# Bojian-Wei/Non-IID-Distributed-Learning-with-Optimal-Mixture-Weights

Hardware: AMD Instinct MI355X
Metric: client-rounds/sec (whole node) (higher is better)
Workload: dtype f32; 1 GPU; config 2: fedavg, 100 clients x 512 rows, RFF D=2048, C=10, E=2, B=32, 10000 test rows, round=1880, parallel clients; algo=fedavg, clients_total=100, clients_per_gpu=100, rows_per_client=512, D=2048, C=10, epochs=2, batch=32, test_rows=10000, parallelism=clients1

## Files before the change

### non-iid-distributed-learning-with-optimal-mixture-weights_amd/_lib.py

```python
import ctypes as C
import os

import torch

from . import LIB_PATH

_c_f32p = C.POINTER(C.c_float)
_SIGS = {
    'fs_abi_version': (C.c_int, []),
    'fs_last_error': (C.c_char_p, []),
    'fs_tuning_size': (C.c_int64, []),
    'fs_set_tuning': (C.c_int, [C.c_void_p]),
    'fs_set_thread_tuning': (C.c_int, [C.c_void_p]),
    'fs_get_tuning': (C.c_int, [C.c_void_p]),
    'fs_get_process_tuning': (C.c_int, [C.c_void_p]),
    'fs_get_thread_tuning': (C.c_int, [C.c_void_p]),
    'fs_randperm_batch': (C.c_int, [C.c_void_p, C.c_void_p, C.c_void_p, C.c_int64, C.c_void_p, C.c_int]),
    'fs_libsvm_scan': (C.c_int, [C.c_char_p, C.c_void_p, C.c_void_p, C.c_void_p]),
    'fs_libsvm_read': (C.c_int, [C.c_char_p, C.c_int64, C.c_int64, C.c_int, C.c_void_p, C.c_void_p, C.c_int]),
    'fs_randperm_device': (C.c_int, [C.c_void_p, C.c_void_p, C.c_void_p, C.c_int64, C.c_int64, C.c_void_p,
                                     C.c_void_p, C.c_void_p]),
    'fs_local_train_plan': (C.c_int, [C.c_int, C.c_int, C.c_int, C.c_int, C.c_int64, C.c_int64, C.c_int,
                                      C.c_int, C.c_void_p, C.c_void_p]),
    'fs_local_train': (C.c_int, [C.c_void_p, C.c_int64, C.c_void_p, C.c_void_p, C.c_void_p, C.c_void_p,
                                 C.c_int, C.c_int, C.c_int, C.c_int, C.c_float, C.c_float, C.c_int,
                                 C.c_float, C.c_int, C.c_int, C.c_void_p, C.c_void_p, C.c_void_p,
                                 C.c_int, C.c_void_p, C.c_int64, C.c_void_p]),
    'fs_local_train_mse': (C.c_int, [C.c_void_p, C.c_int64, C.c_void_p, C.c_void_p, C.c_void_p, C.c_void_p,
                                     C.c_int, C.c_int, C.c_int, C.c_float, C.c_float, C.c_int, C.c_float, C.c_int,
                                     C.c_int, C.c_void_p, C.c_void_p, C.c_void_p, C.c_void_p]),
    'fs_aggregate': (C.c_int, [C.c_void_p, C.c_int64, C.c_void_p, C.c_int, C.c_int64, C.c_void_p,
                               C.c_void_p, C.c_int64, C.c_int, C.c_void_p]),
    'fs_aggregate_sel': (C.c_int, [C.c_void_p, C.c_int64, C.c_void_p, C.c_void_p, C.c_int, C.c_int64, C.c_void_p,
                                   C.c_void_p, C.c_int64, C.c_int, C.c_void_p]),
    'fs_aggregate_nova': (C.c_int, [C.c_void_p, C.c_int64, C.c_void_p, C.c_void_p, C.c_void_p, C.c_float, C.c_float,
                                    C.c_int, C.c_void_p, C.c_int, C.c_int64, C.c_void_p, C.c_void_p, C.c_int64,
                                    C.c_int, C.c_void_p]),
    'fs_local_train_scaffold': (C.c_int, [C.c_void_p, C.c_int64, C.c_void_p, C.c_void_p, C.c_void_p, C.c_void_p,
                                          C.c_int, C.c_int, C.c_int, C.c_int, C.c_float, C.c_float, C.c_int,
                                          C.c_void_p, C.c_void_p, C.c_void_p, C.c_void_p, C.c_void_p, C.c_void_p]),
    'fs_aggregate_scaffold': (C.c_int, [C.c_void_p, C.c_int64, C.c_void_p, C.c_void_p, C.c_void_p, C.c_float, C.c_int,
                                        C.c_int64, C.c_void_p, C.c_void_p, C.c_void_p, C.c_int64, C.c_int, C.c_void_p]),
    'fs_plan_set_scaffold': (C.c_int, [C.c_void_p, C.c_int, C.c_void_p, C.c_void_p, C.c_void_p, C.c_float]),
    'fs_aggregate_opt': (C.c_int, [C.c_void_p, C.c_int64, C.c_void_p, C.c_void_p, C.c_int, C.c_float, C.c_float,
                                   C.c_float, C.c_float, C.c_float, C.c_float, C.c_int, C.c_int64, C.c_void_p,
                                   C.c_void_p, C.c_void_p, C.c_void_p, C.c_int64, C.c_int, C.c_void_p]),
    'fs_plan_set_server_opt': (C.c_int, [C.c_void_p, C.c_int, C.c_void_p, C.c_void_p, C.c_float, C.c_float, C.c_float,
                                         C.c_float, C.c_float, C.c_float]),
    'fs_eval_ws_doubles': (C.c_int64, [C.c_int]),
    'fs_eval': (C.c_int, [C.c_void_p, C.c_int64, C.c_void_p, C.c_int, C.c_void_p, C.c_int, C.c_void_p,
                          C.c_void_p, C.c_void_p]),
    'fs_eval_mse': (C.c_int, [C.c_void_p, C.c_int64, C.c_void_p, C.c_int, C.c_void_p, C.c_void_p, C.c_void_p,
                              C.c_void_p]),
    'fs_z_eval_block_rows': (C.c_int, []),
    'fs_z_eval_ws_doubles': (C.c_int64, [C.c_int, C.c_int]),
    'fs_z_eval_add': (C.c_int, [C.c_void_p, C.c_void_p, C.c_int, C.c_int, C.c_int, C.c_int, C.c_int, C.c_void_p,
                                C.c_int64, C.c_void_p]),
    'fs_z_eval_add_mse': (C.c_int, [C.c_void_p, C.c_void_p, C.c_int, C.c_int, C.c_int, C.c_int, C.c_void_p,
                                    C.c_int64, C.c_void_p]),
    'fs_z_eval_finish': (C.c_int, [C.c_void_p, C.c_int64, C.c_int, C.c_int, C.c_void_p, C.c_void_p]),
    'fs_eval_clients_ws_doubles': (C.c_int64, [C.c_int64, C.c_int]),
    'fs_eval_clients': (C.c_int, [C.c_void_p, C.c_int64, C.c_void_p, C.c_void_p, C.c_void_p, C.c_int, C.c_void_p,
                                  C.c_int64, C.c_int, C.c_void_p, C.c_void_p, C.c_int64, C.c_void_p]),
    'fs_eval_clients_mse': (C.c_int, [C.c_void_p, C.c_int64, C.c_void_p, C.c_void_p, C.c_void_p, C.c_int, C.c_void_p,
                                      C.c_int64, C.c_void_p, C.c_void_p, C.c_int64, C.c_void_p]),
    'fs_mix_z': (C.c_int, [C.c_void_p, C.c_void_p, C.c_int64, C.c_int, C.c_int, C.c_int, C.c_void_p,
                           C.c_void_p]),
    'fs_mix_solve_ws_bytes': (C.c_int64, [C.c_int, C.c_int, C.c_int]),
    'fs_mix_solve': (C.c_int, [C.c_void_p, C.c_void_p, C.c_void_p, C.c_int, C.c_int, C.c_int, C.c_int,
                               C.c_int, C.c_float, C.c_float, C.c_void_p, C.c_void_p, C.c_void_p,
                               C.c_void_p, C.c_int64, C.c_void_p]),
    'fs_mix_solve_mse': (C.c_int, [C.c_void_p, C.c_void_p, C.c_void_p, C.c_int, C.c_int, C.c_int, C.c_int,
                                   C.c_float, C.c_float, C.c_void_p, C.c_void_p, C.c_void_p, C.c_void_p, C.c_int64,
                                   C.c_void_p]),
    'fs_mix_solve_blocked': (C.c_int, [C.c_void_p, C.c_int, C.c_void_p, C.c_void_p, C.c_int, C.c_int, C.c_int,
                                       C.c_int, C.c_int, C.c_float, C.c_float, C.c_void_p, C.c_void_p, C.c_void_p,
                                       C.c_void_p, C.c_int64, C.c_void_p]),
    'fs_mix_solve_blocked_covers': (C.c_int, [C.c_int, C.c_int, C.c_int, C.c_int, C.c_int]),
    'fs_mix_solve_last_mode': (C.c_int, []),
    'fs_mix_solve_last_layout': (C.c_int, [C.c_void_p, C.c_void_p]),
    'fs_mix_solve_plan': (C.c_int, [C.c_int, C.c_int, C.c_int, C.c_int, C.c_int, C.c_int, C.c_void_p]),
    'fs_feature_map': (C.c_int, [C.c_void_p, C.c_int64, C.c_void_p, C.c_void_p, C.c_int, C.c_int, C.c_int,
                                 C.c_float, C.c_void_p, C.c_int64, C.c_void_p]),
    'fs_gram': (C.c_int, [C.c_void_p, C.c_int64, C.c_int64, C.c_int, C.c_void_p, C.c_int64, C.c_void_p]),
    'fs_hetero': (C.c_int, [C.c_void_p, C.c_int64, C.c_void_p, C.c_int, C.c_int, C.c_void_p, C.c_int64, C.c_int64,
                            C.c_void_p, C.c_void_p]),
    'fs_plan_desc_size': (C.c_int64, []),
    'fs_plan_create': (C.c_int, [C.c_void_p, C.c_void_p]),
    'fs_plan_destroy': (C.c_int, [C.c_void_p]),
    'fs_plan_shuffle': (C.c_int, [C.c_void_p, C.c_void_p, C.c_int]),
    'fs_plan_round': (C.c_int, [C.c_void_p, C.c_int, C.c_float, C.c_int, C.c_void_p, C.c_void_p]),
    'fs_plan_eval_flush': (C.c_int, [C.c_void_p, C.c_void_p]),
    'fs_plan_shuffle_subset': (C.c_int, [C.c_void_p, C.c_void_p, C.c_void_p, C.c_int, C.c_int]),
    'fs_plan_round_subset': (C.c_int, [C.c_void_p, C.c_int, C.c_float, C.c_int, C.c_void_p, C.c_void_p, C.c_void_p,
                                       C.c_int, C.c_void_p]),
    'fs_plan_set_nova': (C.c_int, [C.c_void_p, C.c_int, C.c_void_p, C.c_float, C.c_float]),
    'fs_local_train_last_kernel': (C.c_int, []),
    'fs_plan_set_shuffle_chunk': (C.c_int, [C.c_void_p, C.c_int]),
    'fs_plan_shuffle_flush': (C.c_int, [C.c_void_p]),
    'fs_plan_eval_blocks': (C.c_int, [C.c_void_p]),
    'fs_timer_create': (C.c_int, [C.c_void_p]),
    'fs_timer_record': (C.c_int, [C.c_void_p, C.c_void_p]),
    'fs_timer_elapsed_ms': (C.c_int, [C.c_void_p, C.c_void_p, C.c_void_p]),
    'fs_timer_destroy': (C.c_int, [C.c_void_p]),
}

EXPORTS = tuple(_SIGS)
ABI_VERSION = 23

PHASE_TRAIN, PHASE_AGGREGATE, PHASE_EVAL, PHASE_EVAL_DEFER = 1, 2, 4, 8
NOVA_REFERENCE, NOVA_UPDATES = 1, 2
OPT_AVGM, OPT_ADAGRAD, OPT_ADAM, OPT_YOGI = 1, 2, 3, 4
OPT_RULES = {'avgm': OPT_AVGM, 'adagrad': OPT_ADAGRAD, 'adam': OPT_ADAM, 'yogi': OPT_YOGI}
G_PAIR = 256
G_TEAMS = 512
LT_KERNELS = {1: 'single', 2: 'split', 3: 'dbuf', 4: 'pair', 5: 'pipe', 6: 'teams', 7: 'mb',
              8: 'wide'}
G_PIPE = 1024
G_WIDE = 2048
ERR_BLOCK = 256
SOLVER_NAMES = {0: 'none', 1: 'reg', 2: 'mc', 3: 'staged', 4: 'global', 5: 'reg2', 6: 'wave', 8: 'quad', 9: 'qmc', 10: 'bin'}
SOLVERS = {v: k for k, v in SOLVER_NAMES.items() if k}


class Tuning(C.Structure):
    _fields_ = [('mix_solver', C.c_int), ('mix_prefetch', C.c_int), ('mix_prefetch_lead', C.c_int),
                ('mix_exact_softmax', C.c_int), ('no_eval_fuse', C.c_int), ('spin_limit', C.c_uint),
                ('inject_timeout', C.c_int), ('train_form', C.c_int),
                ('split_early', C.c_int), ('mix_qmc_lane_clients', C.c_int),
                ('mix_quad_loaders', C.c_int), ('split_teams', C.c_int),
                ('mix_poll_delay', C.c_int), ('split_poll_delay', C.c_int), ('split_pipe', C.c_int),
                ('split_dbuf', C.c_int),
                ('split_mb', C.c_int)]


class PlanDesc(C.Structure):
    _fields_ = [
        ('d_phi', C.c_void_p), ('ld', C.c_int64), ('d_row_off', C.c_void_p), ('d_labels', C.c_void_p),
        ('d_order', C.c_void_p), ('h_n', C.c_void_p),
        ('N', C.c_int), ('C', C.c_int), ('B', C.c_int), ('E', C.c_int), ('G', C.c_int),
        ('d_ws', C.c_void_p), ('ws_bytes', C.c_int64),
        ('chained', C.c_int), ('prox', C.c_int), ('reg', C.c_int), ('mu', C.c_float), ('lam', C.c_float),
        ('d_W_g', C.c_void_p), ('d_W_out', C.c_void_p), ('d_loss_hist', C.c_void_p),
        ('d_p', C.c_void_p), ('d_agg_ws', C.c_void_p), ('agg_ws_floats', C.c_int64), ('agg_chunks', C.c_int),
        ('d_phi_t', C.c_void_p), ('d_labels_t', C.c_void_p), ('n_t', C.c_int), ('d_eval_ws', C.c_void_p),
        ('d_eval_hist', C.c_void_p), ('shuffle_device', C.c_int), ('host_threads', C.c_int),
        ('shuffle_after_train', C.c_int),
        ('loss', C.c_int), ('d_y', C.c_void_p), ('d_y_t', C.c_void_p),
    ]

_lib = None


class FedsimError(RuntimeError):
    pass


def lib():
    global _lib
    if _lib is None:
        path = os.environ.get('FEDSIM_LIB') or LIB_PATH
        if not os.path.exists(path):
            raise FedsimError(
                'libfedsim.so not found at %s -- build it with `python -c "import __graft_entry__ as g; g.build()"` '
                'or `make -C <pkg>/csrc`; there is no CPU fallback' % path)
        h = C.CDLL(path, mode=C.RTLD_GLOBAL)
        for name, (res, args) in _SIGS.items():
            f = getattr(h, name)
            f.restype = res
            f.argtypes = args
        if h.fs_abi_version() != ABI_VERSION:
            raise FedsimError('libfedsim.so ABI %d != %d' % (h.fs_abi_version(), ABI_VERSION))
        if h.fs_tuning_size() != C.sizeof(Tuning):
            raise FedsimError('fs_tuning layout mismatch (%d != %d bytes)' % (h.fs_tuning_size(), C.sizeof(Tuning)))
        if h.fs_plan_desc_size() != C.sizeof(PlanDesc):
            raise FedsimError('fs_plan_desc layout mismatch (%d != %d bytes)' % (h.fs_plan_desc_size(),
                                                                                  C.sizeof(PlanDesc)))
        _lib = h
    return _lib


_randperm_capped = None


def randperm_device_capped():
    global _randperm_capped
    if _randperm_capped is None:
        f = getattr(lib(), '_ZN2fs15randperm_deviceEPKlS1_S1_llPiPjiPv')
        f.restype = C.c_int
        f.argtypes = [C.c_void_p, C.c_void_p, C.c_void_p, C.c_int64, C.c_int64, C.c_void_p, C.c_void_p, C.c_int,
                      C.c_void_p]
        _randperm_capped = f
    return _randperm_capped


def get_tuning():
    t = Tuning()
    check(lib().fs_get_tuning(C.byref(t)), 'fs_get_tuning')
    return {k: getattr(t, k) for k, _ in Tuning._fields_}


def last_mix_layout():
    k, nk = C.c_int(0), C.c_int(0)
    check(lib().fs_mix_solve_last_layout(C.byref(k), C.byref(nk)), 'fs_mix_solve_last_layout')
    return k.value, nk.value


class MixPlan(C.Structure):
    _fields_ = [('solver', C.c_int), ('workgroups', C.c_int), ('lane_clients', C.c_int), ('helpers', C.c_int),
                ('lead', C.c_int), ('poll_delay', C.c_int), ('ws_bytes', C.c_int64)]


def mix_plan(N, C_, n_val, epochs, Bv, blocks=1):
    out = MixPlan()
    check(lib().fs_mix_solve_plan(int(N), int(C_), int(n_val), int(epochs), int(Bv), int(blocks), C.byref(out)),
          'fs_mix_solve_plan')
    return {k: getattr(out, k) for k, _ in MixPlan._fields_}


def get_process_tuning():
    t = Tuning()
    check(lib().fs_get_process_tuning(C.byref(t)), 'fs_get_process_tuning')
    return {k: getattr(t, k) for k, _ in Tuning._fields_}


def get_thread_tuning():
    t = Tuning()
    has = lib().fs_get_thread_tuning(C.byref(t))
    if has < 0:
        check(has, 'fs_get_thread_tuning')
    return {k: getattr(t, k) for k, _ in Tuning._fields_} if has else None


def _merged(base, fields):
    cur = dict(base)
    for k, v in fields.items():
        if k not in cur:
            raise KeyError('fs_tuning has no field %r' % k)
        if k == 'mix_solver' and isinstance(v, str):
            v = 0 if v == 'auto' else SOLVERS[v]
        cur[k] = int(v)
    return cur


def set_tuning(**fields):
    prev = get_process_tuning()
    check(lib().fs_set_tuning(C.byref(Tuning(**_merged(prev, fields)))), 'fs_set_tuning')
    return prev


def set_thread_tuning(fields=None):
    if fields is None:
        check(lib().fs_set_thread_tuning(None), 'fs_set_thread_tuning')
        return
    cur = _merged({k: 0 for k, _ in Tuning._fields_}, fields)
    check(lib().fs_set_thread_tuning(C.byref(Tuning(**cur))), 'fs_set_thread_tuning')


class tuning:

    def __init__(self, **fields):
        self.fields = fields

    def __enter__(self):
        own = get_thread_tuning()
        self.thread_prev = own
        if own is not None:
            set_thread_tuning(_merged(own, self.fields))
        else:
            self.prev = set_tuning(**self.fields)
        return self

    def __exit__(self, *exc):
        if self.thread_prev is not None:
            set_thread_tuning(self.thread_prev)
        else:
            check(lib().fs_set_tuning(C.byref(Tuning(**self.prev))), 'fs_set_tuning')
        return False


def check(status, what):
    if status != 0:
        msg = lib().fs_last_error()
        raise FedsimError('%s failed (%d): %s' % (what, status, msg.decode() if msg else ''))


def ptr(t):
    return None if t is None else C.c_void_p(t.data_ptr())


def stream_ptr(stream=None):
    s = stream if stream is not None else torch.cuda.current_stream()
    return C.c_void_p(s.cuda_stream)


KERNEL_SOURCES = {
    'local_train': ('local_train.hip', 'local_train_split.hip', 'local_train_pair.hip', 'local_train_pipe.hip',
                    'local_train_dbuf.hip', 'split_common.h', 'local_train_forms.h', 'common.h',
                    'eval_rows.h', 'lanes.h'),
    'mix_solve': ('mixture.hip', 'mixture_forms.h', 'common.h', 'lanes.h'),
    'mix_z': ('mix_z.hip', 'common.h'),
    'local_train_wide': ('local_train_wide.hip', 'local_train_wide.h', 'common.h'),
    'local_train_mse': ('local_train_mse.hip', 'mse_rows.h', 'common.h'),
    'mix_solve_mse': ('mixture_mse.hip', 'mse_rows.h', 'common.h'),
    'z_eval': ('z_eval.hip', 'common.h'),
    'aggregate_nova': ('aggregate_nova.hip', 'aggregate.hip', 'aggregate_sel.h', 'finalize.h', 'common.h'),
    'local_train_scaffold': ('local_train_scaffold.hip', 'scaffold.h', 'common.h'),
    'aggregate_scaffold': ('aggregate_scaffold.hip', 'aggregate.hip', 'aggregate_sel.h', 'scaffold.h', 'finalize.h',
                           'common.h'),
    'aggregate_opt': ('aggregate_opt.hip', 'aggregate.hip', 'aggregate_sel.h', 'finalize.h', 'common.h'),
}


def source_revision(kernel=None):
    import hashlib
    import glob
    pkg = os.path.dirname(os.path.abspath(__file__))
    if kernel:
        files = sorted(os.path.join(pkg, 'csrc', f) for f in KERNEL_SOURCES[kernel])
    else:
        files = sorted(glob.glob(os.path.join(pkg, 'csrc', '*.hip')) + glob.glob(os.path.join(pkg, 'csrc', '*.h')))
    h = hashlib.sha256()
    for f in files:
        h.update(os.path.basename(f).encode())
        with open(f, 'rb') as fh:
            h.update(_code_only(fh.read().decode()).encode())
    return h.hexdigest()[:16]


_TOKENS = None


def _code_only(src):
    global _TOKENS
    import re
    if _TOKENS is None:
        _TOKENS = re.compile(r'"(?:\\.|[^"\\])*"|\'(?:\\.|[^\'\\])*\'|//[^\n]*|/\*.*?\*/|\s+|[^"\'/\s]+|/',
                             re.S)
    out = []
    for m in _TOKENS.finditer(src):
        t = m.group(0)
        if t.startswith('//') or t.startswith('/*'):
            out.append(' ')
        elif t.isspace():
            out.append(' ')
        else:
            out.append(t)
    return re.sub(r' +', ' ', ''.join(out)).strip()


class Timer:

    def __init__(self):
        self._ev = C.c_void_p()
        check(lib().fs_timer_create(C.byref(self._ev)), 'fs_timer_create')

    def record(self):
        check(lib().fs_timer_record(self._ev, stream_ptr()), 'fs_timer_record')

    def elapsed_time(self, end):
        ms = C.c_float()
        check(lib().fs_timer_elapsed_ms(self._ev, end._ev, C.byref(ms)), 'fs_timer_elapsed_ms')
        return float(ms.value)

    def __del__(self):
        if getattr(self, '_ev', None) is not None and self._ev.value and _lib is not None:
            _lib.fs_timer_destroy(self._ev)
            self._ev = None
```

### non-iid-distributed-learning-with-optimal-mixture-weights_amd/csrc/randperm.hip

```cpp
#include "common.h"
#include "randperm_geom.h"

namespace fs {

constexpr int MT_N = RP_MT_N, MT_M = 397;
constexpr int RP_THREADS = 64;

__device__ __forceinline__ uint32_t mt_mix(uint32_t a, uint32_t b, uint32_t c) {
  const uint32_t y = (a & 0x80000000u) | (b & 0x7fffffffu);
  return c ^ (y >> 1) ^ ((y & 1u) ? 0x9908b0dfu : 0u);
}

__device__ __forceinline__ uint32_t mt_temper(uint32_t y) {
  y ^= y >> 11;
  y ^= (y << 7) & 0x9d2c5680u;
  y ^= (y << 15) & 0xefc60000u;
  y ^= y >> 18;
  return y;
}

template <bool WG>
__device__ __forceinline__ void rp_sync() {
  if (WG) {
    __syncthreads();
  } else {
    asm volatile("s_waitcnt lgkmcnt(0)" ::: "memory");
    __builtin_amdgcn_wave_barrier();
    asm volatile("" ::: "memory");
  }
}

template <bool WG>
__device__ __forceinline__ void mt_twist(uint32_t* mt, int lane) {
  uint32_t v[4];
#pragma unroll
  for (int k = 0; k < 4; ++k) {
    const int i = lane + 64 * k;
    if (i < MT_N - MT_M) v[k] = mt_mix(mt[i], mt[i + 1], mt[i + MT_M]);
  }
  rp_sync<WG>();
#pragma unroll
  for (int k = 0; k < 4; ++k) {
    const int i = lane + 64 * k;
    if (i < MT_N - MT_M) mt[i] = v[k];
  }
  rp_sync<WG>();
#pragma unroll
  for (int k = 0; k < 4; ++k) {
    const int i = (MT_N - MT_M) + lane + 64 * k;
    if (i < 2 * (MT_N - MT_M)) v[k] = mt_mix(mt[i], mt[i + 1], mt[i + MT_M - MT_N]);
  }
  rp_sync<WG>();
#pragma unroll
  for (int k = 0; k < 4; ++k) {
    const int i = (MT_N - MT_M) + lane + 64 * k;
    if (i < 2 * (MT_N - MT_M)) mt[i] = v[k];
  }
  rp_sync<WG>();
#pragma unroll
  for (int k = 0; k < 3; ++k) {
    const int i = 2 * (MT_N - MT_M) + lane + 64 * k;
    if (i < MT_N - 1) v[k] = mt_mix(mt[i], mt[i + 1], mt[i + MT_M - MT_N]);
  }
  rp_sync<WG>();
#pragma unroll
  for (int k = 0; k < 3; ++k) {
    const int i = 2 * (MT_N - MT_M) + lane + 64 * k;
    if (i < MT_N - 1) mt[i] = v[k];
  }
  rp_sync<WG>();
  if (lane == 0) mt[MT_N - 1] = mt_mix(mt[MT_N - 1], mt[0], mt[MT_M - 1]);
  rp_sync<WG>();
}

__device__ __forceinline__ void rp_contract_broken(int32_t* dst, int n, int lane, int stride, uint32_t* err) {
  for (int i = lane; i < n; i += stride) dst[i] = i;
  if (err && lane == 0) __hip_atomic_store(err, 1u, __ATOMIC_RELAXED, __HIP_MEMORY_SCOPE_AGENT);
}

template <bool IN_LDS, bool WG>
__device__ __forceinline__ void rp_pass(uint32_t* mt, uint32_t* rnd, int32_t* perm_lds,
                                        const int64_t* __restrict__ seeds, const int64_t* __restrict__ ns,
                                        const int64_t* __restrict__ offs, int32_t* __restrict__ out, int64_t max_n,
                                        uint32_t* err, int64_t pass, int lane) {
  const int64_t n64 = ns[pass];
  int32_t* dst = out + offs[pass];
  if (n64 > max_n) {
    rp_contract_broken(dst, (int)n64, lane, RP_THREADS, err);
    return;
  }
  const int n = (int)n64;
  int32_t* perm = IN_LDS ? perm_lds : dst;
  for (int i = lane; i < n; i += RP_THREADS) perm[i] = i;
  if (lane == 0) {
    uint32_t x = (uint32_t)(uint64_t)seeds[pass];
    mt[0] = x;
    for (int i = 1; i < MT_N; ++i) {
      x = 1812433253u * (x ^ (x >> 30)) + (uint32_t)i;
      mt[i] = x;
    }
  }
  rp_sync<WG>();
  for (int i0 = 0; i0 < n - 1; i0 += MT_N) {
    mt_twist<WG>(mt, lane);
    for (int k = lane; k < MT_N; k += RP_THREADS) rnd[k] = mt_temper(mt[k]);
    rp_sync<WG>();
    if (lane == 0) {
      const int i1 = min(n - 1, i0 + MT_N);
      for (int i = i0; i < i1; ++i) {
        const uint32_t z = rnd[i - i0] % (uint32_t)(n - i);
        const int32_t a = perm[i];
        perm[i] = perm[i + z];
        perm[i + z] = a;
      }
    }
    rp_sync<WG>();
  }
  if (IN_LDS)
    for (int i = lane; i < n; i += RP_THREADS) dst[i] = perm[i];
}

template <bool IN_LDS>
__global__ __launch_bounds__(RP_THREADS) void randperm_kernel(const int64_t* __restrict__ seeds,
                                                             const int64_t* __restrict__ ns,
                                                             const int64_t* __restrict__ offs,
                                                             int32_t* __restrict__ out, int64_t max_n,
                                                             uint32_t* err) {
  extern __shared__ __attribute__((aligned(16))) uint32_t smem_rp[];
  uint32_t* mt = smem_rp;
  uint32_t* rnd = mt + MT_N;
  rp_pass<IN_LDS, true>(mt, rnd, reinterpret_cast<int32_t*>(rnd + MT_N), seeds, ns, offs, out, max_n, err,
                        blockIdx.x, threadIdx.x);
}

__global__ __launch_bounds__(RP_THREADS * RP_MAX_WAVES) void randperm_capped_kernel(
    const int64_t* __restrict__ seeds, const int64_t* __restrict__ ns, const int64_t* __restrict__ offs,
    int64_t npasses, int32_t* __restrict__ out, int64_t max_n, uint32_t* err, int region) {
  extern __shared__ __attribute__((aligned(16))) uint32_t smem_rp[];
  const int lane = threadIdx.x & (RP_THREADS - 1);
  const int wave = __builtin_amdgcn_readfirstlane(threadIdx.x / RP_THREADS);
  const int waves = blockDim.x / RP_THREADS;
  uint32_t* mt = smem_rp + (size_t)wave * region;
  uint32_t* rnd = mt + MT_N;
  const int64_t total = (int64_t)gridDim.x * waves;
  for (int64_t pass = (int64_t)blockIdx.x * waves + wave; pass < npasses; pass += total) {
    rp_pass<true, false>(mt, rnd, reinterpret_cast<int32_t*>(rnd + MT_N), seeds, ns, offs, out, max_n, err, pass, lane);
    rp_sync<false>();
  }
}

constexpr int RL_MAXN = 64;

__device__ __forceinline__ void rl_block(int32_t (*perm_s)[RL_MAXN + 1], const int64_t* __restrict__ seeds,
                                         const int64_t* __restrict__ ns, const int64_t* __restrict__ offs,
                                         int64_t npasses, int32_t* __restrict__ out, int max_n, uint32_t* err,
                                         int64_t blk, int lane) {
  const int64_t pass = blk * 64 + lane;
  const bool live = pass < npasses;
  const int n_req = live ? (int)ns[pass] : 0;
  const int n = n_req <= max_n ? n_req : 0;
  if (n_req > max_n && err) __hip_atomic_store(err, 1u, __ATOMIC_RELAXED, __HIP_MEMORY_SCOPE_AGENT);
  int32_t* perm = perm_s[lane];
  uint32_t lo[RL_MAXN], hi[RL_MAXN - 1];
  {
    uint32_t x = live ? (uint32_t)(uint64_t)seeds[pass] : 0u;
    lo[0] = x;
#pragma unroll
    for (int i = 1; i <= MT_M + RL_MAXN - 2; ++i) {
      x = 1812433253u * (x ^ (x >> 30)) + (uint32_t)i;
      if (i < RL_MAXN) lo[i] = x;
      if (i >= MT_M) hi[i - MT_M] = x;
    }
  }
#pragma unroll
  for (int i = 0; i < RL_MAXN; ++i)
    if (i < n) perm[i] = i;
#pragma unroll
  for (int i = 0; i < RL_MAXN - 1; ++i) {
    if (i < n - 1) {
      const uint32_t r = mt_temper(mt_mix(lo[i], lo[i + 1], hi[i]));
      const int z = (int)(r % (uint32_t)(n - i));
      const int32_t a = perm[i];
      perm[i] = perm[i + z];
      perm[i + z] = a;
    }
  }
  if (live) {
    int32_t* dst = out + offs[pass];
    for (int i = 0; i < n; ++i) dst[i] = perm[i];
    for (int i = n; i < n_req; ++i) dst[i] = i;
  }
}

__global__ __launch_bounds__(64) void randperm_lanes_kernel(const int64_t* __restrict__ seeds,
                                                           const int64_t* __restrict__ ns,
                                                           const int64_t* __restrict__ offs, int64_t npasses,
                                                           int32_t* __restrict__ out, int max_n, uint32_t* err) {
  __shared__ int32_t perm_s[64][RL_MAXN + 1];
  rl_block(perm_s, seeds, ns, offs, npasses, out, max_n, err, blockIdx.x, threadIdx.x);
}

__global__ __launch_bounds__(64) void randperm_lanes_capped_kernel(const int64_t* __restrict__ seeds,
                                                                  const int64_t* __restrict__ ns,
                                                                  const int64_t* __restrict__ offs, int64_t npasses,
                                                                  int32_t* __restrict__ out, int max_n,
                                                                  uint32_t* err) {
  __shared__ int32_t perm_s[64][RL_MAXN + 1];
  for (int64_t blk = blockIdx.x; blk * 64 < npasses; blk += gridDim.x)
    rl_block(perm_s, seeds, ns, offs, npasses, out, max_n, err, blk, threadIdx.x);
}

}

namespace fs {

int randperm_device(const int64_t* d_seeds, const int64_t* d_n, const int64_t* d_off, int64_t npasses, int64_t max_n,
                    int32_t* d_out, uint32_t* d_err, int max_blocks, void* stream) {
  FS_REQUIRE(npasses >= 0 && max_n >= 0 && max_n < ((int64_t)1 << 31) && max_blocks >= 0, "bad sizes");
  if (npasses == 0) return FS_OK;
  FS_REQUIRE(d_seeds && d_n && d_off && d_out, "null pointer");
  hipStream_t st = reinterpret_cast<hipStream_t>(stream);
  if (max_n <= RL_MAXN) {
    if (max_blocks > 0)
      hipLaunchKernelGGL(randperm_lanes_capped_kernel, dim3((unsigned)rp_capped_lanes_geom(npasses, max_blocks).blocks),
                         dim3(64), 0, st, d_seeds, d_n, d_off, npasses, d_out, (int)max_n, d_err);
    else
      hipLaunchKernelGGL(randperm_lanes_kernel, dim3((unsigned)((npasses + 63) / 64)), dim3(64), 0, st, d_seeds, d_n,
                         d_off, npasses, d_out, (int)max_n, d_err);
    FS_LAUNCH_CHECK();
    return FS_OK;
  }
  if (max_blocks > 0 && rp_in_lds(max_n)) {
    const RpGeom g = rp_capped_geom(npasses, max_n, max_blocks);
    if (g.lds > 64 * 1024) {
      hipError_t e = hipFuncSetAttribute(reinterpret_cast<const void*>(&randperm_capped_kernel),
                                         hipFuncAttributeMaxDynamicSharedMemorySize, (int)g.lds);
      if (e != hipSuccess) return fail(FS_EHIP, std::string("fs_randperm_device: ") + hipGetErrorString(e));
    }
    hipLaunchKernelGGL(randperm_capped_kernel, dim3((unsigned)g.blocks), dim3(RP_THREADS * g.waves), (size_t)g.lds, st,
                       d_seeds, d_n, d_off, npasses, d_out, max_n, d_err, (int)rp_region_words(max_n, true));
    FS_LAUNCH_CHECK();
    return FS_OK;
  }
  const size_t lds_small = sizeof(uint32_t) * 2 * MT_N;
  const size_t lds_full = lds_small + sizeof(int32_t) * (size_t)max_n;
  if (lds_full <= 160 * 1024) {
    if (lds_full > 64 * 1024) {
      hipError_t e = hipFuncSetAttribute(reinterpret_cast<const void*>(&randperm_kernel<true>),
                                         hipFuncAttributeMaxDynamicSharedMemorySize, (int)lds_full);
      if (e != hipSuccess) return fail(FS_EHIP, std::string("fs_randperm_device: ") + hipGetErrorString(e));
    }
    hipLaunchKernelGGL(randperm_kernel<true>, dim3((unsigned)npasses), dim3(RP_THREADS), lds_full, st, d_seeds, d_n,
                       d_off, d_out, max_n, d_err);
  } else {
    hipLaunchKernelGGL(randperm_kernel<false>, dim3((unsigned)npasses), dim3(RP_THREADS), lds_small, st, d_seeds, d_n,
                       d_off, d_out, max_n, d_err);
  }
  FS_LAUNCH_CHECK();
  return FS_OK;
}

}

using namespace fs;

extern "C" int fs_randperm_device(const int64_t* d_seeds, const int64_t* d_n, const int64_t* d_off, int64_t npasses,
                                  int64_t max_n, int32_t* d_out, uint32_t* d_err, void* stream) {
  return fs::randperm_device(d_seeds, d_n, d_off, npasses, max_n, d_out, d_err, 0, stream);
}
```

Before: 387,400 client-rounds/s.

## Parallelize Fisher-Yates shuffle via swap-chain resolution across wave lanes

For permutations that fit within one Mersenne Twister block in LDS, the serial lane-0 Fisher-Yates swap loop is replaced by a parallel resolution. Each lane computes its swap target, uses atomicMax and ballots to find the last writer per slot, then follows the swap chains with pointer jumping to produce the same permutation. The serial path also folds the modulo into the parallel fill, and the capped kernel now interleaves passes across blocks rather than waves. A standalone resolve kernel and optional timestamp probes are added. The cost is extra LDS traffic and a more intricate algorithm whose output must match the sequential shuffle exactly.

Result: no change. 386,200 client-rounds/s (-0.3%).

```diff
diff --git a/non-iid-distributed-learning-with-optimal-mixture-weights_amd/_lib.py b/non-iid-distributed-learning-with-optimal-mixture-weights_amd/_lib.py
--- a/non-iid-distributed-learning-with-optimal-mixture-weights_amd/_lib.py
+++ b/non-iid-distributed-learning-with-optimal-mixture-weights_amd/_lib.py
@@ -194,6 +194,19 @@
     return _randperm_capped
 
 
+_randperm_resolve = None
+
+
+def randperm_resolve_device():
+    global _randperm_resolve
+    if _randperm_resolve is None:
+        f = getattr(lib(), '_ZN2fs23randperm_resolve_deviceEPKiPKlS3_lPiPjiPv')
+        f.restype = C.c_int
+        f.argtypes = [C.c_void_p, C.c_void_p, C.c_void_p, C.c_int64, C.c_void_p, C.c_void_p, C.c_int, C.c_void_p]
+        _randperm_resolve = f
+    return _randperm_resolve
+
+
 def get_tuning():
     t = Tuning()
     check(lib().fs_get_tuning(C.byref(t)), 'fs_get_tuning')
diff --git a/non-iid-distributed-learning-with-optimal-mixture-weights_amd/csrc/randperm.hip b/non-iid-distributed-learning-with-optimal-mixture-weights_amd/csrc/randperm.hip
--- a/non-iid-distributed-learning-with-optimal-mixture-weights_amd/csrc/randperm.hip
+++ b/non-iid-distributed-learning-with-optimal-mixture-weights_amd/csrc/randperm.hip
@@ -76,6 +76,98 @@
 __device__ __forceinline__ void rp_contract_broken(int32_t* dst, int n, int lane, int stride, uint32_t* err) {
   for (int i = lane; i < n; i += stride) dst[i] = i;
   if (err && lane == 0) __hip_atomic_store(err, 1u, __ATOMIC_RELAXED, __HIP_MEMORY_SCOPE_AGENT);
+}
+
+#ifdef FS_RP_STAMPS
+#define RP_STAMP_BEGIN()                                                                   \
+  unsigned long long stamp_prev;                                                           \
+  asm volatile("s_memtime %0\n\ts_waitcnt lgkmcnt(0)" : "=s"(stamp_prev)::"memory");
+#define RP_STAMP(k)                                                                        \
+  {                                                                                        \
+    __builtin_amdgcn_sched_barrier(0);                                                     \
+    unsigned long long t_;                                                                 \
+    asm volatile("s_memtime %0\n\ts_waitcnt lgkmcnt(0)" : "=s"(t_)::"memory");            \
+    __builtin_amdgcn_sched_barrier(0);                                                     \
+    if (err && blockIdx.x == 0 && threadIdx.x == 0) {                                      \
+      err[8 + 2 * (k)] += (uint32_t)(t_ - stamp_prev);                                     \
+      err[9 + 2 * (k)] += 1u;                                                              \
+    }                                                                                      \
+    stamp_prev = t_;                                                                       \
+  }
+#else
+#define RP_STAMP_BEGIN()
+#define RP_STAMP(k)
+#endif
+
+constexpr int RP_RESOLVE_N = MT_N;
+constexpr int RP_RESOLVE_SLOTS = (RP_RESOLVE_N + RP_THREADS - 1) / RP_THREADS;
+
+template <bool WG>
+__device__ __forceinline__ void rp_resolve(int32_t* last, int32_t* ptr, int32_t* __restrict__ dst,
+                                           const int32_t (&tk)[RP_RESOLVE_SLOTS], int n, int lane) {
+  int32_t l[RP_RESOLVE_SLOTS], top[RP_RESOLVE_SLOTS], a[RP_RESOLVE_SLOTS], b[RP_RESOLVE_SLOTS];
+  constexpr int SPARE = MT_N;
+#pragma unroll
+  for (int k = 0; k < RP_RESOLVE_SLOTS; ++k) {
+    const int i = lane + RP_THREADS * k;
+    last[i < n ? i : SPARE] = -1;
+  }
+#pragma unroll
+  for (int k = 0; k < RP_RESOLVE_SLOTS; ++k) {
+    const int i = lane + RP_THREADS * k;
+    int32_t* at = &last[i < n ? tk[k] : SPARE];
+    asm volatile("" ::: "memory");
+    l[k] = *at;
+    atomicMax(at, i);
+    top[k] = *at;
+  }
+  asm volatile("" ::: "memory");
+#pragma unroll
+  for (int k = 0; k < RP_RESOLVE_SLOTS; ++k) {
+    const int i = lane + RP_THREADS * k;
+    a[k] = last[i < n ? i : SPARE];
+  }
+  rp_sync<WG>();
+#pragma unroll
+  for (int k = 0; k < RP_RESOLVE_SLOTS; ++k) {
+    const int i = lane + RP_THREADS * k;
+    const bool live = i < n;
+    if (!live) l[k] = -1;
+    uint64_t cand = __ballot(live && top[k] != i);
+    while (cand) {
+      const int j = __builtin_ctzll(cand);
+      cand &= cand - 1;
+      const int32_t tj = __builtin_amdgcn_readlane(tk[k], j);
+      if (tj == tk[k] && j < lane) l[k] = RP_THREADS * k + j;
+    }
+    const int32_t lf = a[k];
+    a[k] = lf == i ? (l[k] >= 0 ? l[k] : i) : (lf >= 0 ? lf : i);
+    if (!live) a[k] = 0;
+    if (live) ptr[i] = a[k];
+  }
+  for (int span = 1; span < n; span <<= 1) {
+#pragma unroll
+    for (int k = 0; k < RP_RESOLVE_SLOTS; ++k) b[k] = ptr[a[k]];
+    asm volatile("" ::: "memory");
+    bool moved = false;
+#pragma unroll
+    for (int k = 0; k < RP_RESOLVE_SLOTS; ++k) {
+      if (b[k] != a[k]) {
+        ptr[lane + RP_THREADS * k] = b[k];
+        a[k] = b[k];
+        moved = true;
+      }
+    }
+    if (!__any(moved)) break;
+  }
+  rp_sync<WG>();
+#pragma unroll
+  for (int k = 0; k < RP_RESOLVE_SLOTS; ++k) b[k] = ptr[max(l[k], 0)];
+#pragma unroll
+  for (int k = 0; k < RP_RESOLVE_SLOTS; ++k) {
+    const int i = lane + RP_THREADS * k;
+    if (i < n) dst[i] = l[k] >= 0 ? b[k] : tk[k];
+  }
 }
 
 template <bool IN_LDS, bool WG>
@@ -90,8 +182,15 @@
     return;
   }
   const int n = (int)n64;
+  if (n <= 1) {
+    if (n == 1 && lane == 0) dst[0] = 0;
+    return;
+  }
+  RP_STAMP_BEGIN();
+  const bool resolve = IN_LDS && n <= RP_RESOLVE_N;
   int32_t* perm = IN_LDS ? perm_lds : dst;
-  for (int i = lane; i < n; i += RP_THREADS) perm[i] = i;
+  if (!resolve)
+    for (int i = lane; i < n; i += RP_THREADS) perm[i] = i;
   if (lane == 0) {
     uint32_t x = (uint32_t)(uint64_t)seeds[pass];
     mt[0] = x;
@@ -101,23 +200,48 @@
     }
   }
   rp_sync<WG>();
+  RP_STAMP(0);
+  if (resolve) {
+    mt_twist<WG>(mt, lane);
+    int32_t tk[RP_RESOLVE_SLOTS];
+#pragma unroll
+    for (int k = 0; k < RP_RESOLVE_SLOTS; ++k) {
+      const int i = lane + RP_THREADS * k;
+      tk[k] = i == n - 1 ? i : -1;
+      if (RP_THREADS * k < n - 1) {
+        const uint32_t r = mt_temper(mt[min(i, MT_N - 1)]);
+        if (i < n - 1) tk[k] = i + (int32_t)(r % (uint32_t)max(n - i, 1));
+      }
+    }
+    rp_sync<WG>();
+    RP_STAMP(1);
+    rp_resolve<WG>(reinterpret_cast<int32_t*>(mt), perm_lds, dst, tk, n, lane);
+    RP_STAMP(2);
+    return;
+  }
   for (int i0 = 0; i0 < n - 1; i0 += MT_N) {
     mt_twist<WG>(mt, lane);
-    for (int k = lane; k < MT_N; k += RP_THREADS) rnd[k] = mt_temper(mt[k]);
+    for (int k = lane; k < MT_N; k += RP_THREADS) {
+      const int i = i0 + k;
+      if (i < n - 1) rnd[k] = (uint32_t)i + mt_temper(mt[k]) % (uint32_t)(n - i);
+    }
     rp_sync<WG>();
+    RP_STAMP(1);
     if (lane == 0) {
       const int i1 = min(n - 1, i0 + MT_N);
       for (int i = i0; i < i1; ++i) {
-        const uint32_t z = rnd[i - i0] % (uint32_t)(n - i);
+        const uint32_t t = rnd[i - i0];
         const int32_t a = perm[i];
-        perm[i] = perm[i + z];
-        perm[i + z] = a;
+        perm[i] = perm[t];
+        perm[t] = a;
       }
     }
     rp_sync<WG>();
+    RP_STAMP(2);
   }
   if (IN_LDS)
     for (int i = lane; i < n; i += RP_THREADS) dst[i] = perm[i];
+  RP_STAMP(3);
 }
 
 template <bool IN_LDS>
@@ -143,9 +267,40 @@
   uint32_t* mt = smem_rp + (size_t)wave * region;
   uint32_t* rnd = mt + MT_N;
   const int64_t total = (int64_t)gridDim.x * waves;
-  for (int64_t pass = (int64_t)blockIdx.x * waves + wave; pass < npasses; pass += total) {
+  for (int64_t pass = (int64_t)wave * gridDim.x + blockIdx.x; pass < npasses; pass += total) {
     rp_pass<true, false>(mt, rnd, reinterpret_cast<int32_t*>(rnd + MT_N), seeds, ns, offs, out, max_n, err, pass, lane);
     rp_sync<false>();
+  }
+}
+
+template <bool WG>
+__global__ __launch_bounds__(WG ? RP_THREADS : RP_THREADS * RP_MAX_WAVES) void randperm_resolve_kernel(
+    const int32_t* __restrict__ targets, const int64_t* __restrict__ ns, const int64_t* __restrict__ offs,
+    int64_t npasses, int32_t* __restrict__ out, uint32_t* err, int region) {
+  extern __shared__ __attribute__((aligned(16))) uint32_t smem_rp[];
+  const int lane = threadIdx.x & (RP_THREADS - 1);
+  const int wave = __builtin_amdgcn_readfirstlane(threadIdx.x / RP_THREADS);
+  const int waves = blockDim.x / RP_THREADS;
+  int32_t* last = reinterpret_cast<int32_t*>(smem_rp) + (size_t)wave * region;
+  int32_t* ptr = last + 2 * MT_N;
+  const int64_t total = (int64_t)gridDim.x * waves;
+  for (int64_t pass = (int64_t)wave * gridDim.x + blockIdx.x; pass < npasses; pass += total) {
+    const int64_t n64 = ns[pass];
+    int32_t* dst = out + offs[pass];
+    if (n64 > RP_RESOLVE_N) {
+      rp_contract_broken(dst, (int)n64, lane, RP_THREADS, err);
+      continue;
+    }
+    const int n = (int)n64;
+    int32_t tk[RP_RESOLVE_SLOTS];
+#pragma unroll
+    for (int k = 0; k < RP_RESOLVE_SLOTS; ++k) {
+      const int i = lane + RP_THREADS * k;
+      tk[k] = i == n - 1 ? i : -1;
+      if (i < n - 1) tk[k] = min(max(targets[offs[pass] + i], i), n - 1);
+    }
+    rp_resolve<WG>(last, ptr, dst, tk, n, lane);
+    rp_sync<WG>();
   }
 }
 
@@ -260,6 +415,30 @@
   return FS_OK;
 }
 
+int randperm_resolve_device(const int32_t* d_t, const int64_t* d_n, const int64_t* d_off, int64_t npasses,
+                            int32_t* d_out, uint32_t* d_err, int max_blocks, void* stream) {
+  FS_REQUIRE(npasses >= 0 && max_blocks >= 0, "bad sizes");
+  if (npasses == 0) return FS_OK;
+  FS_REQUIRE(d_t && d_n && d_off && d_out, "null pointer");
+  hipStream_t st = reinterpret_cast<hipStream_t>(stream);
+  const int region = (int)rp_region_words(RP_RESOLVE_N, true);
+  if (max_blocks > 0) {
+    const RpGeom g = rp_capped_geom(npasses, RP_RESOLVE_N, max_blocks);
+    if (g.lds > 64 * 1024) {
+      hipError_t e = hipFuncSetAttribute(reinterpret_cast<const void*>(&randperm_resolve_kernel<false>),
+                                         hipFuncAttributeMaxDynamicSharedMemorySize, (int)g.lds);
+      if (e != hipSuccess) return fail(FS_EHIP, std::string("fs::randperm_resolve_device: ") + hipGetErrorString(e));
+    }
+    hipLaunchKernelGGL(randperm_resolve_kernel<false>, dim3((unsigned)g.blocks), dim3(RP_THREADS * g.waves),
+                       (size_t)g.lds, st, d_t, d_n, d_off, npasses, d_out, d_err, region);
+  } else {
+    hipLaunchKernelGGL(randperm_resolve_kernel<true>, dim3((unsigned)npasses), dim3(RP_THREADS),
+                       sizeof(uint32_t) * (size_t)region, st, d_t, d_n, d_off, npasses, d_out, d_err, region);
+  }
+  FS_LAUNCH_CHECK();
+  return FS_OK;
+}
+
 }
 
 using namespace fs;
```
